# arthurlirui/IRON

Hardware: AMD Instinct MI355X
Metric: Mrays/s sphere-trace+GGX shade, drv/dragon 800x800 (synthetic S0) (higher is better)
Workload: dtype f32

## Files before the change

iron_amd/csrc/getall_rev.hip:

```cpp
#include <stdlib.h>
#include "mlp_h2_rev.h"
#include "h2_setup.h"
#include "shade_args.h"

namespace iron {

template <int T>
__device__ __forceinline__ void pe_contract(const f32x16& g, const float* pe, int half, float& gx, float& gy, float& gz) {
#pragma unroll
    for (int r = 0; r < 16; ++r) {
        const int s = 16 * T + r;
        if (s == 0) {
            if (half) gy += g[r]; else gx += g[r];
        } else if (s == 1) {
            if (!half) gz += g[r];
        } else if (s < 2 + 3 * kSdfPeLevels) {
            const int k = (s - 2) / 3, c = (s - 2) % 3;
            const float f = (float)(1 << k);
            const float v = (half ? f : -f) * pe[s] * g[r];
            if (c == 0) gx += v; else if (c == 1) gy += v; else gz += v;
        }
    }
}

#ifndef IRON_REV_FEAT_NT
#define IRON_REV_FEAT_NT 0
#endif
#ifdef IRON_REV_DEBUG
#define IRON_REV_DUMP(L, BUF)                                                                                              \
    if (dbg == (L) && a.feat_rows && ok) {                                                                                 \
        _Pragma("unroll") for (int t_ = 0; t_ < kHidTiles; ++t_)                                                           \
            _Pragma("unroll") for (int r_ = 0; r_ < 16; ++r_) {                                                            \
                const int s_ = r_ >> 3, j_ = r_ & 7;                                                                       \
                const float v_ = (float)BUF[t_].h[s_][j_] + (float)BUF[t_].l[s_][j_] * kLoInv;                             \
                a.feat_rows[(size_t)li * kHidden + 32 * t_ + (r_ & 3) + 8 * (r_ >> 2) + 4 * half] = v_;                    \
            }                                                                                                              \
    }
#define IRON_REV_DBG_PARAM , int dbg
#else
#define IRON_REV_DUMP(L, BUF)
#define IRON_REV_DBG_PARAM
#endif

__global__ __launch_bounds__(256, 1) void k_sdf_getall_rev_h2(H2StreamDev hs, H2Meta m, GradArgs a, char* __restrict__ park IRON_REV_DBG_PARAM) {
    extern __shared__ __attribute__((aligned(16))) char smem[];
    char* lds = smem;
    const int lane = threadIdx.x & 63;
    const int half = lane >> 5;
    const int wave = __builtin_amdgcn_readfirstlane(threadIdx.x >> 6);
    Ring ring;
    h2_setup(hs, lds, ring);
    ParkBuf pb;
    pb.rsrc = __builtin_amdgcn_make_buffer_rsrc(park + (size_t)blockIdx.x * kParkBytesPerWg, 0, kParkBytesPerWg, 0x00020000);
    pb.voff = lane * 16;
    const int count = a.count_ptr ? *a.count_ptr : a.count;
    const int n_tiles = (count + kTile - 1) / kTile;
    const int n_groups = (n_tiles + 3) / 4;
    const bool want_feat = (a.feat_packed != nullptr) || (a.feat_rows != nullptr);
    const char* bias = lds + kLdsBias;

    for (int g = blockIdx.x; g < n_groups; g += gridDim.x) {
        const int tile = 4 * g + wave;
        const int li = tile * kTile + (lane & 31);
        const bool ok = li < count;
        const int src = ok ? (a.list ? a.list[li] : li) : 0;
        float px = 0.f, py = 0.f, pz = 0.f;
        if (ok) { px = a.x[3 * (size_t)src]; py = a.x[3 * (size_t)src + 1]; pz = a.x[3 * (size_t)src + 2]; }
        const float sx = px * m.scale, sy = py * m.scale, sz = pz * m.scale;

        TileFrag X[kHidTiles], Y[kHidTiles];
        f32x16 hf[kHidTiles];
        HeadFrag hd;
        {
            float pe[kHeadSlots];
#pragma unroll
            for (int i = 0; i < kHeadSlots; ++i) pe[i] = 0.0f;
            head_fill<kSdfPeLevels>(sx, sy, sz, half, pe);
            split_head(pe, hd);
        }
#pragma unroll
        for (int to = 0; to < kHidTiles; ++to) {
            ring.sync();
            const RingStep st = ring.step();
            f32x16 a_hi = zero16(), a_lo = zero16();
            step_head(st.rd, bias, st.wr, st.src, st.hidden, wave, lane, to, true, hd, a_hi, a_lo);
            f32x16 h, P;
            softplus_park_tile(h2_combine(a_hi, a_lo), h, P);
            park_store_tile(pb, park_off(0, to, wave), P);
            split_tile(h, X[to]);
        }
        for (int l = 1; l < 7; l += 2) {
            h2_layer_x<kModeFwd, false, false>(ring, bias + l * 1024, hd, lane, X, Y, hf, pb, l);
            if (l + 1 == 4) h2_layer_x<kModeFwd, true, false>(ring, bias + (l + 1) * 1024, hd, lane, Y, X, hf, pb, l + 1);
            else h2_layer_x<kModeFwd, false, false>(ring, bias + (l + 1) * 1024, hd, lane, Y, X, hf, pb, l + 1);
        }
        h2_layer_x<kModeFwd, false, true>(ring, bias + 7 * 1024, hd, lane, X, Y, hf, pb, 7);
        {
            const float s = (row_dot_lds(lds + kLdsRows, hf, half) + m.b_last) / m.scale;
            if (ok && lane < 32 && a.sdf_out) a.sdf_out[li] = s;
        }
#pragma unroll
        for (int t = 0; t < kHidTiles; ++t) split_tile(hf[t], X[t]);
        {
            const char* fb = bias + 8 * 1024;
            float* dst = (a.feat_packed && tile < n_tiles) ? a.feat_packed + (size_t)tile * (kHidTiles * 16 * 64) : nullptr;
#pragma unroll
            for (int to = 0; to < kHidTiles; ++to) {
                const f32x16 o = h2_plain_tile(ring, fb, lane, to, true, X, pb);
                if (want_feat && !(IRON_REV_ABL & 4)) {
                    if (dst) feat_store_tile<IRON_REV_FEAT_NT != 0>(dst, to, lane, o);
#ifdef IRON_REV_DEBUG
                    if (a.feat_rows && ok && dbg < 0) {
#else
                    if (a.feat_rows && ok) {
#endif
#pragma unroll
                        for (int r = 0; r < 16; ++r) a.feat_rows[(size_t)li * kHidden + 32 * to + (r & 3) + 8 * (r >> 2) + 4 * half] = o[r];
                    }
                }
            }
        }
#pragma unroll
        for (int t = 0; t < kHidTiles; ++t) {
            const f32x16 P = park_load_tile(pb, park_off(7, t, wave));
            f32x16 d = lds_half_tile(lds + kLdsRows, t, half);
#pragma unroll
            for (int i = 0; i < 16; ++i) d[i] *= sigma_from_park(P[i]);
            split_tile(d, Y[t]);
        }
        float gx = 0.f, gy = 0.f, gz = 0.f;
        float pe[kHeadSlots];
#pragma unroll
        for (int i = 0; i < kHeadSlots; ++i) pe[i] = 0.0f;
        if (!(IRON_REV_ABL & 8)) head_fill<kSdfPeLevels>(sx, sy, sz, half, pe);
        IRON_REV_DUMP(7, Y)
        h2_layer_x<kModeBwd, false, false>(ring, bias, hd, lane, Y, X, hf, pb, 6);
        IRON_REV_DUMP(6, X)
        h2_layer_x<kModeBwd, false, false>(ring, bias, hd, lane, X, Y, hf, pb, 5);
        IRON_REV_DUMP(5, Y)
        h2_layer_x<kModeBwd, false, false>(ring, bias, hd, lane, Y, X, hf, pb, 4);
        IRON_REV_DUMP(4, X)
        h2_layer_x<kModeBwd, false, false>(ring, bias, hd, lane, X, Y, hf, pb, 3);
        IRON_REV_DUMP(3, Y)
        {
            const f32x16 g0 = h2_plain_tile(ring, bias, lane, 0, false, X, pb);
            pe_contract<0>(g0, pe, half, gx, gy, gz);
            const f32x16 g1 = h2_plain_tile(ring, bias, lane, 1, false, X, pb);
            pe_contract<1>(g1, pe, half, gx, gy, gz);
        }
        h2_layer_x<kModeBwd, false, false>(ring, bias, hd, lane, Y, X, hf, pb, 2);
        IRON_REV_DUMP(2, X)
        h2_layer_x<kModeBwd, false, false>(ring, bias, hd, lane, X, Y, hf, pb, 1);
        IRON_REV_DUMP(1, Y)
        h2_layer_x<kModeBwd, false, false>(ring, bias, hd, lane, Y, X, hf, pb, 0);
        IRON_REV_DUMP(0, X)
        {
            const f32x16 g0 = h2_plain_tile(ring, bias, lane, 0, false, X, pb);
            pe_contract<0>(g0, pe, half, gx, gy, gz);
            const f32x16 g1 = h2_plain_tile(ring, bias, lane, 1, false, X, pb);
            pe_contract<1>(g1, pe, half, gx, gy, gz);
        }
        gx += __shfl_xor(gx, 32, 64);
        gy += __shfl_xor(gy, 32, 64);
        gz += __shfl_xor(gz, 32, 64);
        if (ok && lane < 32 && a.grad_out) {
            a.grad_out[3 * (size_t)li] = gx; a.grad_out[3 * (size_t)li + 1] = gy; a.grad_out[3 * (size_t)li + 2] = gz;
        }
    }
    ring.drain();
}

size_t getall_rev_park_bytes(int64_t n_points) {
    const int64_t groups = (n_points + 127) / 128;
    const int64_t cus = cu_total();
    return (size_t)(groups < cus ? (groups > 0 ? groups : 1) : cus) * kParkBytesPerWg;
}

bool getall_rev_usable(const iron_net* sdf) {
    static int on = -1;
    if (on < 0) {
        const char* e = getenv("IRON_GETALL");
        on = (e && e[0] == 'f') ? 0 : 1;
    }
    return on == 1 && h2_sdf_usable(sdf) && sdf->h2_rev_blob != nullptr;
}

int launch_sdf_getall_rev(const iron_net* sdf, const GradArgs& a, int64_t max_tiles, void* park, size_t park_bytes, hipStream_t st) {
    static bool attr = false;
    if (!attr) {
        IRON_HIP_TRY(hipFuncSetAttribute((const void*)k_sdf_getall_rev_h2, hipFuncAttributeMaxDynamicSharedMemorySize, kLdsH2Total));
        attr = true;
    }
    H2Meta m;
    m.n_hidden_layers = sdf->sdf.n_hidden_layers; m.skip_layer = sdf->sdf.skip_layer; m.scale = sdf->sdf.scale; m.b_last = sdf->sdf.b_last;
    const int64_t groups = (max_tiles + 3) / 4;
    const int64_t cus = cu_budget();
    int64_t grid = groups < cus ? (groups > 0 ? groups : 1) : cus;
    const int64_t cap = (int64_t)(park_bytes / kParkBytesPerWg);
    if (!park || cap < 1) return IRON_ERR_WORKSPACE;
    if (grid > cap) grid = cap;
    if (((uintptr_t)park & 15) != 0) return IRON_ERR_BAD_ARG;
    ProfScope ps(IRON_PROF_SDF_GRAD, st);
#ifdef IRON_REV_DEBUG
    const char* de = getenv("IRON_REV_DEBUG_LAYER");
    hipLaunchKernelGGL(k_sdf_getall_rev_h2, dim3((unsigned)grid), dim3(256), kLdsH2Total, st, sdf->h2_rev, m, a, (char*)park, de ? atoi(de) : -1);
#else
    hipLaunchKernelGGL(k_sdf_getall_rev_h2, dim3((unsigned)grid), dim3(256), kLdsH2Total, st, sdf->h2_rev, m, a, (char*)park);
#endif
    IRON_HIP_TRY(hipGetLastError());
    return IRON_OK;
}

}
```

iron_amd/csrc/mlp_core.h:

```cpp
#pragma once
#include "iron_common.h"

namespace iron {

typedef float f32x16 __attribute__((ext_vector_type(16)));
typedef float f32x4 __attribute__((ext_vector_type(4)));
typedef int i32x4 __attribute__((ext_vector_type(4)));

template <bool NT = false>
__device__ __forceinline__ void feat_store_tile(float* __restrict__ tile_base, int t, int lane, const f32x16& o) {
    f32x4* p = reinterpret_cast<f32x4*>(tile_base) + (size_t)(t * 4) * 64 + lane;
#pragma unroll
    for (int q = 0; q < 4; ++q) {
        f32x4 v;
        v[0] = o[4 * q]; v[1] = o[4 * q + 1]; v[2] = o[4 * q + 2]; v[3] = o[4 * q + 3];
        if (NT) __builtin_nontemporal_store(v, p + q * 64);
        else p[q * 64] = v;
    }
}
__device__ __forceinline__ f32x16 feat_load_tile(const float* __restrict__ tile_base, int t, int lane) {
    const float4* p = reinterpret_cast<const float4*>(tile_base) + (size_t)(t * 4) * 64 + lane;
    f32x16 v;
#pragma unroll
    for (int q = 0; q < 4; ++q) {
        const float4 x = p[q * 64];
        v[4 * q] = x.x; v[4 * q + 1] = x.y; v[4 * q + 2] = x.z; v[4 * q + 3] = x.w;
    }
    return v;
}

#ifndef IRON_WQ_DEPTH
#define IRON_WQ_DEPTH 4
#endif

__device__ __forceinline__ f32x16 mfma32(float a, float b, f32x16 c) {
    return __builtin_amdgcn_mfma_f32_32x32x2f32(a, b, c, 0, 0, 0);
}

struct WStream {
    __amdgpu_buffer_rsrc_t rsrc;
    int v_lane;
    int v_half;
    __device__ __forceinline__ void init(const void* blob, uint32_t bytes, int lane) {
        rsrc = __builtin_amdgcn_make_buffer_rsrc(const_cast<void*>(blob), 0, (int)bytes, 0x00020000);
        v_lane = lane * 16;
        v_half = (lane >> 5) * 64;
    }
    __device__ __forceinline__ f32x4 frag(uint32_t s_off) const {
        return __builtin_bit_cast(f32x4, __builtin_amdgcn_raw_buffer_load_b128(rsrc, v_lane, (int)s_off, 0));
    }
    __device__ __forceinline__ f32x4 half_row(uint32_t s_off) const {
        return __builtin_bit_cast(f32x4, __builtin_amdgcn_raw_buffer_load_b128(rsrc, v_half, (int)s_off, 0));
    }
};

template <bool FAST>
__device__ __forceinline__ float softplus100(float z) {
    if constexpr (FAST) {
        const float e = __builtin_amdgcn_exp2f(__builtin_fabsf(z) * -144.26950408889634f);
        return __builtin_fmaf(__builtin_amdgcn_logf(1.0f + e), 0.0069314718055994531f, fmaxf(z, 0.0f));
    } else {
        const float t = z * 100.0f;
        const float s = log1pf(expf(t)) / 100.0f;
        return t > 20.0f ? z : s;
    }
}

__device__ __forceinline__ float softplus100_grad(float z) {
    const float t = z * 100.0f;
    const float s = 1.0f / (1.0f + expf(-t));
    return t > 20.0f ? 1.0f : s;
}

__device__ __forceinline__ f32x16 load_half_tile(const WStream& ws, uint32_t base, int tile) {
    const uint32_t o = base + (uint32_t)tile * 128u;
    const f32x4 b0 = ws.half_row(o), b1 = ws.half_row(o + 16), b2 = ws.half_row(o + 32), b3 = ws.half_row(o + 48);
    f32x16 v;
    v[0] = b0.x; v[1] = b0.y; v[2] = b0.z; v[3] = b0.w;
    v[4] = b1.x; v[5] = b1.y; v[6] = b1.z; v[7] = b1.w;
    v[8] = b2.x; v[9] = b2.y; v[10] = b2.z; v[11] = b2.w;
    v[12] = b3.x; v[13] = b3.y; v[14] = b3.z; v[15] = b3.w;
    return v;
}

template <int LEVELS>
__device__ __forceinline__ void head_fill(float vx, float vy, float vz, int half, float* slots) {
    slots[0] = half ? vy : vx;
    slots[1] = half ? 0.0f : vz;
#pragma unroll
    for (int k = 0; k < LEVELS; ++k) {
        const float f = (float)(1 << k);
        float s, c;
        sincosf(vx * f, &s, &c); slots[2 + 3 * k + 0] = half ? c : s;
        sincosf(vy * f, &s, &c); slots[2 + 3 * k + 1] = half ? c : s;
        sincosf(vz * f, &s, &c); slots[2 + 3 * k + 2] = half ? c : s;
    }
}

template <int LEVELS>
__device__ __forceinline__ void head_fill4(float vx, float vy, float vz, float vw, int half, float* slots) {
    slots[0] = half ? vy : vx;
    slots[1] = half ? vw : vz;
    const float v[4] = {vx, vy, vz, vw};
#pragma unroll
    for (int k = 0; k < LEVELS; ++k) {
        const float f = (float)(1 << k);
#pragma unroll
        for (int c = 0; c < 4; ++c) {
            float s, cs;
            sincosf(v[c] * f, &s, &cs);
            slots[2 + 4 * k + c] = half ? cs : s;
        }
    }
}

__device__ __forceinline__ void mfma_quad(const f32x4& a0, const f32x4& a1, float b0, float b1, float b2, float b3,
                                          f32x16& acc0, f32x16& acc1) {
    acc0 = mfma32(a0.x, b0, acc0);
    acc1 = mfma32(a1.x, b0, acc1);
    acc0 = mfma32(a0.y, b1, acc0);
    acc1 = mfma32(a1.y, b1, acc1);
    acc0 = mfma32(a0.z, b2, acc0);
    acc1 = mfma32(a1.z, b2, acc1);
    acc0 = mfma32(a0.w, b3, acc0);
    acc1 = mfma32(a1.w, b3, acc1);
}

template <int NQ>
__device__ __forceinline__ void dense_head_pair(const WStream& ws, uint32_t base, int pair, const float* head,
                                                f32x16& acc0, f32x16& acc1) {
    const uint32_t o = base + (uint32_t)pair * (NQ * 2048u);
    constexpr int kChunk = NQ <= 6 ? NQ : 6;
#pragma unroll
    for (int q0 = 0; q0 < NQ; q0 += kChunk) {
        f32x4 a0[kChunk], a1[kChunk];
#pragma unroll
        for (int q = 0; q < kChunk; ++q) {
            if (q0 + q < NQ) {
                a0[q] = ws.frag(o + (q0 + q) * 2048u);
                a1[q] = ws.frag(o + (q0 + q) * 2048u + 1024u);
            }
        }
#pragma unroll
        for (int q = 0; q < kChunk; ++q) {
            if (q0 + q < NQ)
                mfma_quad(a0[q], a1[q], head[4 * (q0 + q)], head[4 * (q0 + q) + 1], head[4 * (q0 + q) + 2], head[4 * (q0 + q) + 3],
                          acc0, acc1);
        }
    }
}

struct WQueue {
    static constexpr int D = IRON_WQ_DEPTH;
    f32x4 a0[D], a1[D];
    __device__ __forceinline__ void prime(const WStream& ws, uint32_t base) {
#pragma unroll
        for (int d = 0; d < D; ++d) {
            a0[d] = ws.frag(base + d * 2048u);
            a1[d] = ws.frag(base + d * 2048u + 1024u);
        }
    }
};

#ifndef IRON_SCHED_MASK
#define IRON_SCHED_MASK 0x6
#endif

template <int PAIR>
__device__ __forceinline__ void dense_hidden_pair(const WStream& ws, uint32_t base, WQueue& wq,
                                                  const f32x16 (&in)[kHidTiles], f32x16& acc0, f32x16& acc1) {
#pragma unroll
    for (int s = 0; s < 32; ++s) {
        constexpr int D = WQueue::D;
        const int g = PAIR * 32 + s;
        const int slot = g % D;
        const f32x4 x0 = wq.a0[slot], x1 = wq.a1[slot];
        wq.a0[slot] = ws.frag(base + (uint32_t)(g + D) * 2048u);
        wq.a1[slot] = ws.frag(base + (uint32_t)(g + D) * 2048u + 1024u);
// ... 128 lines not shown
```

iron_amd/csrc/mlp_h2.h:

```cpp
#pragma once
#include "iron_common.h"
#include "mlp_core.h"
#include "lds_dma.h"

#ifndef IRON_H2_STAMP
#define IRON_H2_STAMP 0
#endif
#ifndef IRON_H2_ASM_DMA
#define IRON_H2_ASM_DMA 0
#endif
#ifndef IRON_H2_FRAG_AHEAD
#define IRON_H2_FRAG_AHEAD 1
#endif
#ifndef IRON_H2_RING_AHEAD
#define IRON_H2_RING_AHEAD 3
#endif
#ifndef IRON_H2_SPREAD
#define IRON_H2_SPREAD 1
#endif
#ifndef IRON_H2_ABL
#define IRON_H2_ABL 0
#endif
#ifndef IRON_H2_ROT_ISSUE
#define IRON_H2_ROT_ISSUE 0
#endif

namespace iron {

typedef _Float16 half8 __attribute__((ext_vector_type(8)));
typedef _Float16 half2v __attribute__((ext_vector_type(2)));

constexpr int kRingSlots = 4;
constexpr int kSlotBytes = 32768;
constexpr int kRingBytes = kRingSlots * kSlotBytes;
constexpr int kRingAhead = IRON_H2_RING_AHEAD;
constexpr int kLoadsPerSlot = 8;
constexpr float kLoScale = 2048.0f;
constexpr float kLoInv = 1.0f / 2048.0f;
constexpr int kHeadSlots = 24;
constexpr int kHeadKSteps = 3;

constexpr int kLdsRing = 0;
constexpr int kLdsBias = kRingBytes;
constexpr int kLdsBiasBytes = 9 * 1024;
constexpr int kLdsRows = kLdsBias + kLdsBiasBytes;
constexpr int kLdsRowsBytes = 3 * 1024;
constexpr int kLdsTable = kLdsRows + kLdsRowsBytes;
constexpr int kLdsTableBytes = 1024;
constexpr int kLdsMisc = kLdsTable + kLdsTableBytes;
constexpr int kLdsMiscBytes = 256;
constexpr int kLdsH2Total = kLdsMisc + kLdsMiscBytes;

constexpr int kLdsStamp = kLdsH2Total;
constexpr int kStampSteps = 72;
constexpr int kStampFirst = 144;
constexpr int kLdsStampBytes = 4 * kStampSteps * 8 * 8;
__device__ __forceinline__ void h2_stamp(unsigned long long* rec, int k) {
#if IRON_H2_STAMP
    if (rec) {
        const unsigned long long t = __builtin_readcyclecounter();
        if ((threadIdx.x & 63) == 0) rec[k] = t;
    }
    __builtin_amdgcn_sched_barrier(0);
#endif
}

__device__ __forceinline__ f32x16 mfma_h(half8 a, half8 b, f32x16 c) {
    return __builtin_amdgcn_mfma_f32_32x32x16_f16(a, b, c, 0, 0, 0);
}

typedef _Float16 f16x2 __attribute__((ext_vector_type(2)));
typedef unsigned int u32x4 __attribute__((ext_vector_type(4)));

__device__ __forceinline__ void split2(float x0, float x1, unsigned& hi, unsigned& lo) {
    f16x2 h;
    h[0] = (_Float16)x0;
    h[1] = (_Float16)x1;
    f16x2 l;
    l[0] = (_Float16)((x0 - (float)h[0]) * kLoScale);
    l[1] = (_Float16)((x1 - (float)h[1]) * kLoScale);
    hi = __builtin_bit_cast(unsigned, h);
    lo = __builtin_bit_cast(unsigned, l);
}

struct TileFrag {
    half8 h[2];
    half8 l[2];
};

__device__ __forceinline__ void split8(const float* v, half8& h, half8& l) {
    u32x4 hh, ll;
#pragma unroll
    for (int i = 0; i < 4; ++i) {
        unsigned a, b;
        split2(v[2 * i], v[2 * i + 1], a, b);
        hh[i] = a;
        ll[i] = b;
    }
    h = __builtin_bit_cast(half8, hh);
    l = __builtin_bit_cast(half8, ll);
}

__device__ __forceinline__ void split_tile(const f32x16& v, TileFrag& t) {
#pragma unroll
// ... 468 lines not shown
                                                const HeadFrag* hd2 = nullptr, const float* __restrict__ init = nullptr) {
    static_assert(!INIT || HEAD > 0, "the partial sums are added on top of the head product");
    static_assert(!(LAST && DEFER), "the last layer ends in f32 tiles");
    const int wave = ring.wave;
    f32x16 acc[2][2];
    TileFrag dummy_out;
    f32x16 dummy_hf;
#define IRON_H2_TILE(TO)                                                                                                   \
    if constexpr ((TO) < NT) {                                                                                             \
        constexpr int P = (TO) & 1, Q = P ^ 1;                                                                             \
        acc[P][0] = zero16();                                                                                              \
        acc[P][1] = zero16();                                                                                              \
        f32x16 part;                                                                                                       \
        if constexpr (INIT) {                                                                                              \
            _Pragma("unroll") for (int r = 0; r < 16; ++r) part[r] = init[((TO) * 16 + r) * 64 + lane];                    \
        }                                                                                                                  \
        if constexpr (HEAD >= 1) {                                                                                         \
            ring.sync();                                                                                                   \
            const RingStep sh = ring.step();                                                                               \
            step_head(sh.rd, bias, sh.wr, sh.src, sh.hidden, wave, lane, TO, true, hd, acc[P][0], acc[P][1]);              \
        }                                                                                                                  \
        if constexpr (HEAD >= 2) {                                                                                         \
            ring.sync();                                                                                                   \
            const RingStep sh = ring.step();                                                                               \
            step_head(sh.rd, bias, sh.wr, sh.src, sh.hidden, wave, lane, TO, false, *hd2, acc[P][0], acc[P][1]);           \
        }                                                                                                                  \
        if constexpr (INIT) {                                                                                              \
            _Pragma("unroll") for (int r = 0; r < 16; ++r) acc[P][0][r] += part[r];                                        \
        }                                                                                                                  \
        ring.sync();                                                                                                       \
        const RingStep st = ring.step();                                                                                   \
        if constexpr ((TO) == 0 && CARRY)                                                                                  \
            step_hidden<FAST, 1, ACT, true>(st.rd, bias, st.wr, st.src, st.hidden, wave, lane, TO, !HEAD, in, acc[P][0],   \
                                            acc[P][1], c_hi, c_lo, dummy_out, dummy_hf, st.rec);                           \
        else if constexpr ((TO) == 0)                                                                                      \
            step_hidden<FAST, 0, ACT>(st.rd, bias, st.wr, st.src, st.hidden, wave, lane, TO, !HEAD, in, acc[P][0], acc[P][1],   \
                                 acc[Q][0], acc[Q][1], dummy_out, dummy_hf, st.rec);                                       \
        else if constexpr (LAST)                                                                                           \
            step_hidden<FAST, 2, ACT>(st.rd, bias, st.wr, st.src, st.hidden, wave, lane, TO, !HEAD, in, acc[P][0], acc[P][1],   \
                                 acc[Q][0], acc[Q][1], dummy_out, hf[(TO) > 0 ? (TO) - 1 : 0], st.rec);                    \
        else                                                                                                               \
            step_hidden<FAST, 1, ACT>(st.rd, bias, st.wr, st.src, st.hidden, wave, lane, TO, !HEAD, in, acc[P][0], acc[P][1],   \
                                 acc[Q][0], acc[Q][1], out[(TO) > 0 ? (TO) - 1 : 0], dummy_hf, st.rec);                    \
    }
    IRON_H2_TILE(0) IRON_H2_TILE(1) IRON_H2_TILE(2) IRON_H2_TILE(3)
    IRON_H2_TILE(4) IRON_H2_TILE(5) IRON_H2_TILE(6) IRON_H2_TILE(7)
#undef IRON_H2_TILE
    static_assert(NT % 2 == 0 && NT >= 2 && NT <= kHidTiles, "the last tile sits in accumulator set 1");
    if constexpr (DEFER) {
        c_hi = acc[1][0];
        c_lo = acc[1][1];
    } else if constexpr (ACT == 0) {
        if constexpr (LAST) hf[NT - 1] = softplus_tile<FAST>(h2_combine(acc[1][0], acc[1][1]));
        else h2_epilogue_split<FAST>(acc[1][0], acc[1][1], out[NT - 1]);
    } else if constexpr (ACT == 1) {
        if constexpr (LAST) hf[NT - 1] = relu_tile_nan(h2_combine(acc[1][0], acc[1][1]));
        else split_tile(relu_tile_nan(h2_combine(acc[1][0], acc[1][1])), out[NT - 1]);
    } else {
        if constexpr (LAST) hf[NT - 1] = h2_combine(acc[1][0], acc[1][1]);
        else split_tile(h2_combine(acc[1][0], acc[1][1]), out[NT - 1]);
    }
}

__device__ __forceinline__ float row_dot_lds(const char* __restrict__ row, const f32x16 (&h)[kHidTiles], int half) {
    float s = 0.0f;
#pragma unroll
    for (int t = 0; t < kHidTiles; ++t) {
        const f32x16 w = lds_half_tile(row, t, half);
#pragma unroll
        for (int r = 0; r < 16; ++r) s = fmaf(w[r], h[t][r], s);
    }
    return s + __shfl_xor(s, 32, 64);
}

template <bool FAST, bool DEFER_TILES = true>
__device__ __forceinline__ void sdf_hidden_stack_h2(Ring& ring, const char* lds, int n_hidden_layers, int skip_layer,
                                                    float scale, float x, float y, float z, int lane,
                                                    f32x16 (&hf)[kHidTiles]) {
    const int half = lane >> 5;
    const int wave = ring.wave;
    float pe[kHeadSlots];
#pragma unroll
    for (int i = 0; i < kHeadSlots; ++i) pe[i] = 0.0f;
    head_fill<kSdfPeLevels>(x * scale, y * scale, z * scale, half, pe);
    HeadFrag hd;
    split_head(pe, hd);

    TileFrag X[kHidTiles], Y[kHidTiles];
#pragma unroll
    for (int to = 0; to < kHidTiles; ++to) {
        ring.sync();
        const RingStep st = ring.step();
        f32x16 a_hi = zero16(), a_lo = zero16();
        step_head(st.rd, lds + kLdsBias, st.wr, st.src, st.hidden, wave, lane, to, true, hd, a_hi, a_lo);
        h2_epilogue_split<FAST>(a_hi, a_lo, X[to]);
    }
    f32x16 c_hi, c_lo;
    constexpr bool D = DEFER_TILES;
    for (int l = 1; l + 1 < n_hidden_layers - 1; l += 2) {
        const char* bias_a = lds + kLdsBias + l * 1024;
        const char* bias_b = bias_a + 1024;
        if (l == 1) h2_hidden_layer<FAST, false, false, 0, false, D>(ring, bias_a, hd, lane, X, Y, hf, c_hi, c_lo);
        else h2_hidden_layer<FAST, false, false, 0, D, D>(ring, bias_a, hd, lane, X, Y, hf, c_hi, c_lo);
        if (l + 1 == skip_layer) h2_hidden_layer<FAST, true, false, 0, D, D>(ring, bias_b, hd, lane, Y, X, hf, c_hi, c_lo);
        else h2_hidden_layer<FAST, false, false, 0, D, D>(ring, bias_b, hd, lane, Y, X, hf, c_hi, c_lo);
    }
    h2_hidden_layer<FAST, false, true, 0, D, false>(ring, lds + kLdsBias + (n_hidden_layers - 1) * 1024, hd, lane, X, Y, hf, c_hi, c_lo);
}

#ifndef IRON_H1_NO_EPI
#define IRON_H1_NO_EPI 0
#endif
constexpr int kH1PointTiles = 2;

struct Epi1State {
    float z[16], e[16];
    u32x4 oh[2];
};

constexpr int kEpi1Ops = 104;
constexpr int kEpi1OpsF32 = 96;

template <bool F32>
__device__ __forceinline__ void epi1_op(Epi1State& st, int op, const f32x16& p) {
    constexpr float kC1 = 144.26950408889634f;
    constexpr float kC2 = 0.0069314718055994531f;
    constexpr int kHalf = F32 ? 48 : 52;
    const int h = op / kHalf, lo = op % kHalf;
#if IRON_H1_NO_EPI
    if (lo >= 48) {
        const int q = 4 * h + lo - 48;
        st.oh[q >> 2][q & 3] = __builtin_bit_cast(unsigned, cvt_pk_rn(p[2 * q], p[2 * q + 1]));
    }
    if (lo >= 40 && lo < 48) st.z[8 * h + lo - 40] = p[8 * h + lo - 40];
    return;
#endif
    if (lo >= 48) {
        const int q = 4 * h + lo - 48;
        unsigned u = __builtin_bit_cast(unsigned, cvt_pk_rn(st.z[2 * q], st.z[2 * q + 1]));
        pin1u(u);
        st.oh[q >> 2][q & 3] = u;
        return;
    }
    const int stage = lo >> 3, i = 8 * h + (lo & 7);
    if (stage == 0) { st.e[i] = __builtin_fabsf(p[i]) * -kC1; pin1(st.e[i]); }
    else if (stage == 1) { st.e[i] = __builtin_amdgcn_exp2f(st.e[i]); pin1(st.e[i]); }
    else if (stage == 2) { st.e[i] = 1.0f + st.e[i]; pin1(st.e[i]); }
    else if (stage == 3) { st.e[i] = __builtin_amdgcn_logf(st.e[i]); pin1(st.e[i]); }
    else if (stage == 4) { st.z[i] = relu_med3(p[i]); pin1(st.z[i]); }
    else { st.z[i] = __builtin_fmaf(st.e[i], kC2, st.z[i]); pin1(st.z[i]); }
}

struct TileH {
    half8 h[2];
};

struct HeadH {
    half8 h[kHeadKSteps];
};

__device__ __forceinline__ void tile_from_epi(const Epi1State& es, TileH& t) {
#pragma unroll
    for (int s = 0; s < 2; ++s) t.h[s] = __builtin_bit_cast(half8, es.oh[s]);
}

__device__ __forceinline__ void row_dot_tile(const char* __restrict__ row, int t, int half, const float* z, float& s) {
    const f32x16 w = lds_half_tile(row, t, half);
#pragma unroll
    for (int r = 0; r < 16; ++r) s = fmaf(w[r], z[r], s);
}

#ifndef IRON_H1_FRAG_AHEAD
#define IRON_H1_FRAG_AHEAD 1
#endif
constexpr int kH1Ahead = IRON_H1_FRAG_AHEAD;
static_assert(kH1Ahead == 1 || kH1Ahead == 2, "IRON_H1_FRAG_AHEAD: 1 or 2");
struct H1Pre {
    half8 f[kH1Ahead];
};

__device__ __forceinline__ const char* h1_slot(Ring& ring, H1Pre& pre, int lane) {
    ring.sync();
    ring.b_take = __builtin_amdgcn_readfirstlane(ring.b_take);
    const RingStep st = ring.step();
#pragma unroll
// ... 230 lines not shown
```

iron_amd/csrc/shade.hip:

```cpp
#include "mlp_h2.h"
#include "h2_setup.h"
#include "ggx_core.h"
#include "shade_args.h"

namespace iron {

#ifndef IRON_FAST_SOFTPLUS
#define IRON_FAST_SOFTPLUS 1
#endif
constexpr bool kFastActS = IRON_FAST_SOFTPLUS != 0;

template <bool FAST>
__device__ __forceinline__ void softplus100_both(float z, float& h, float& s) {
    if constexpr (FAST) {
        const float u = __builtin_amdgcn_exp2f(__builtin_fabsf(z) * -144.26950408889634f);
        const float w = 1.0f + u;
        h = __builtin_fmaf(__builtin_amdgcn_logf(w), 0.0069314718055994531f, fmaxf(z, 0.0f));
        s = (z >= 0.0f ? 1.0f : u) * __builtin_amdgcn_rcpf(w);
    } else {
        const float t = z * 100.0f;
        const float e = expf(t);
        const float l = log1pf(e) / 100.0f;
        const float sg = e / (e + 1.0f);
        const bool lin = t > 20.0f;
// ... 66 lines not shown
    {                                                                                               \
        f32x16 a0 = is_value ? load_half_tile(ws, bb, 2 * P) : zero_tile();                         \
        f32x16 a1 = is_value ? load_half_tile(ws, bb, 2 * P + 1) : zero_tile();                     \
        if (with_head) dense_head_pair<kSdfHeadQuads>(ws, hb, P, head, a0, a1);                     \
        if (l > 0) dense_hidden_pair<P>(ws, wb, wq, h, a0, a1);                                     \
        if (is_value) {                                                                             \
            _Pragma("unroll") for (int r = 0; r < 16; ++r) {                                        \
                float hv, sv;                                                                       \
                softplus100_both<kFastActS>(a0[r], hv, sv);                                         \
                a0[r] = hv;                                                                         \
                sbuf[((2 * P) * 16 + r) * 64 + lane] = sv;                                          \
                softplus100_both<kFastActS>(a1[r], hv, sv);                                         \
                a1[r] = hv;                                                                         \
                sbuf[((2 * P + 1) * 16 + r) * 64 + lane] = sv;                                      \
            }                                                                                       \
        }                                                                                           \
        o[2 * P] = a0;                                                                              \
        o[2 * P + 1] = a1;                                                                          \
    }
            IRON_GPAIR(0) IRON_GPAIR(1) IRON_GPAIR(2) IRON_GPAIR(3)
#undef IRON_GPAIR
            __syncthreads();
            if (!is_value) {
#pragma unroll
                for (int t = 0; t < kHidTiles; ++t)
#pragma unroll
                    for (int r = 0; r < 16; ++r) o[t][r] *= sbuf[(t * 16 + r) * 64 + lane];
            }
#pragma unroll
            for (int t = 0; t < kHidTiles; ++t) h[t] = o[t];
        }

        if (is_value) {
            const float s = (row_dot(ws, net.w_last, h) + net.b_last) / net.scale;
            if (ok && lane < 32 && a.sdf_out) a.sdf_out[li] = s;
            if ((a.feat_packed || a.feat_rows) && net.w_feat) {
                f32x16 o[kHidTiles];
                WQueue wf;
                wf.prime(ws, net.w_feat);
                hidden_layer<IdentityAct, 1>(ws, net.w_feat, net.b_feat, false, 0u, nullptr, wf, h, o, IdentityAct());
                if (a.feat_packed) {
                    float* dst = a.feat_packed + (size_t)tile * kSBufFloats;
#pragma unroll
                    for (int t = 0; t < kHidTiles; ++t) feat_store_tile(dst, t, lane, o[t]);
                }
                if (a.feat_rows && ok) {
#pragma unroll
                    for (int t = 0; t < kHidTiles; ++t)
#pragma unroll
                        for (int r = 0; r < 16; ++r)
                            a.feat_rows[(size_t)li * kHidden + 32 * t + (r & 3) + 8 * (r >> 2) + 4 * half] = o[t][r];
                }
            }
        } else {
            const float g = row_dot(ws, net.w_last, h);
            if (ok && lane < 32 && a.grad_out) a.grad_out[3 * (size_t)li + axis] = g;
        }
        __syncthreads();
    }
}

constexpr int kLdsSbuf = kLdsH2Total;
constexpr int kLdsGradTotal = kLdsH2Total + 8192;

#if defined(IRON_GRAD_VARIANT) && (IRON_GRAD_VARIANT & 1)
#define IRON_GRAD_ACT(Z, H, S) { H = (Z); S = 1.0f; }
#else
#define IRON_GRAD_ACT(Z, H, S) softplus100_both<kFastActS>(Z, H, S)
#endif

__device__ __forceinline__ void lds_publish_barrier() {
    asm volatile("s_waitcnt lgkmcnt(0)" ::: "memory");
    __builtin_amdgcn_s_barrier();
}

__device__ __forceinline__ float sdf_value_or_tangent_h2(Ring& ring, char* lds, float* sbuf, const H2Meta& m, float px, float py,
                                                         float pz, bool is_value, int axis, int wave, int lane,
                                                         TileFrag (&in)[kHidTiles], TileFrag (&out)[kHidTiles]) {
    const int half = lane >> 5;
    const float sx = px * m.scale, sy = py * m.scale, sz = pz * m.scale;
    float head[kHeadSlots];
#pragma unroll
    for (int i = 0; i < kHeadSlots; ++i) head[i] = 0.0f;
    if (is_value) head_fill<kSdfPeLevels>(sx, sy, sz, half, head);
    else head_fill_tangent<kSdfPeLevels>(sx, sy, sz, axis, half, head);
    HeadFrag hd;
    split_head(head, hd);
    TileFrag dummy_out;
    f32x16 dummy_hf;
    f32x16 p_hi = zero16(), p_lo = zero16();
    for (int l = 0; l < m.n_hidden_layers; ++l) {
        const bool last = (l == m.n_hidden_layers - 1);
        const bool with_head = (l == 0) || (l == m.skip_layer);
        const char* bias = lds + kLdsBias + l * 1024;
        if (l > 0) {
#pragma unroll
            for (int t = 0; t < kHidTiles; ++t) in[t] = out[t];
        }
#define IRON_GTILE(TO)                                                                                                  \
    {                                                                                                                   \
        f32x16 a_hi = zero16(), a_lo = zero16();                                                                        \
        if (with_head) {                                                                                                \
            ring.sync();                                                                                                \
            const RingStep sh = ring.step();                                                                            \
            step_head(sh.rd, bias, sh.wr, sh.src, sh.hidden, wave, lane, TO, false, hd, a_hi, a_lo);                    \
        }                                                                                                               \
        if (l > 0) {                                                                                                    \
            ring.sync();                                                                                                \
            const RingStep st = ring.step();                                                                            \
            step_hidden<kFastActS, 0>(st.rd, bias, st.wr, st.src, st.hidden, wave, lane, TO, false, in, a_hi, a_lo,     \
                                      a_hi, a_lo, dummy_out, dummy_hf);                                                 \
        }                                                                                                               \
        if (is_value) {                                                                                                 \
             \
             \
            f32x16 zt = h2_combine(a_hi, a_lo);                                                                         \
            const f32x16 bt = lds_half_tile(bias, TO, half);                                                            \
            float* sb = sbuf + ((TO) & 1) * (16 * 64);                                                                  \
            _Pragma("unroll") for (int r = 0; r < 16; ++r) {                                                            \
                float hv, sv;                                                                                           \
                IRON_GRAD_ACT(zt[r] + bt[r], hv, sv);                                                                   \
                zt[r] = hv;                                                                                             \
                sb[r * 64 + lane] = sv;                                                                                 \
            }                                                                                                           \
            asm volatile("s_waitcnt lgkmcnt(0)" ::: "memory");                                                          \
            if (last) out[TO] = __builtin_bit_cast(TileFrag, zt);                                                       \
            else split_tile(zt, out[TO]);                                                                               \
        } else {                                                                                                        \
             \
            if ((TO) > 0) IRON_GTANGENT_FINISH((TO) - 1)                                                                \
            p_hi = a_hi;                                                                                                \
            p_lo = a_lo;                                                                                                \
        }                                                                                                               \
    }
#define IRON_GTANGENT_FINISH(T)                                                                                         \
    {                                                                                                                   \
        f32x16 zt = h2_combine(p_hi, p_lo);                                                                             \
        const float* sb = sbuf + ((T) & 1) * (16 * 64);                                                                 \
        _Pragma("unroll") for (int r = 0; r < 16; ++r) zt[r] *= sb[r * 64 + lane];                                      \
        if (last) out[T] = __builtin_bit_cast(TileFrag, zt);                                                            \
        else split_tile(zt, out[T]);                                                                                    \
    }
        IRON_GTILE(0) IRON_GTILE(1) IRON_GTILE(2) IRON_GTILE(3) IRON_GTILE(4) IRON_GTILE(5) IRON_GTILE(6) IRON_GTILE(7)
        lds_publish_barrier();
        if (!is_value) IRON_GTANGENT_FINISH(7)
#undef IRON_GTANGENT_FINISH
#undef IRON_GTILE
    }
    f32x16 hf[kHidTiles];
#pragma unroll
    for (int t = 0; t < kHidTiles; ++t) hf[t] = __builtin_bit_cast(f32x16, out[t]);
    const float d = row_dot_lds(lds + kLdsRows, hf, half);
    return is_value ? (d + m.b_last) / m.scale : d;
}

__global__ __launch_bounds__(256, 1) void k_sdf_grad_h2(H2StreamDev hs, H2Meta m, GradArgs a) {
    extern __shared__ __attribute__((aligned(16))) char smem[];
    char* lds = smem;
    const int lane = threadIdx.x & 63;
    const int half = lane >> 5;
    const int wave = __builtin_amdgcn_readfirstlane(threadIdx.x >> 6);
    const bool is_value = wave == 0;
    const int axis = wave - 1;
    Ring ring;
    h2_setup(hs, lds, ring);
    float* sbuf = reinterpret_cast<float*>(lds + kLdsSbuf);
    const int count = a.count_ptr ? *a.count_ptr : a.count;
// ... 170 lines not shown
        if (ok) {
            px = a.points[3 * (size_t)pi]; py = a.points[3 * (size_t)pi + 1]; pz = a.points[3 * (size_t)pi + 2];
            if (a.normals) { nx = a.normals[3 * (size_t)ai]; ny = a.normals[3 * (size_t)ai + 1]; nz = a.normals[3 * (size_t)ai + 2]; }
            if (a.normalise) {
                const float nn = sqrtf((nx * nx + ny * ny) + nz * nz) + 1e-10f;
                nx = nx / nn; ny = ny / nn; nz = nz / nn;
            }
            if (a.neg_normal_view) { vx = -nx; vy = -ny; vz = -nz; }
            else if (a.view) { vx = a.view[3 * (size_t)ai]; vy = a.view[3 * (size_t)ai + 1]; vz = a.view[3 * (size_t)ai + 2]; }
        }
        float head[4 * NQ];
#pragma unroll
        for (int i = 0; i < 4 * NQ; ++i) head[i] = 0.0f;
        int base = 0;
        head_fill<LP>(px, py, pz, half, head + base);
        base += head_slots(LP);
        if constexpr (HAS_VIEW) { head_fill<LV>(vx, vy, vz, half, head + base); base += head_slots(LV); }
        if constexpr (HAS_NRM) { head_fill<0>(nx, ny, nz, half, head + base); base += 2; }

        f32x16 h[kHidTiles];
        load_feature_tiles(a, tile, ai, ok, lane, half, h);

        WQueue wq;
        wq.prime(ws, net.w_feat0);
        for (int l = 0, blk = 0; l < net.n_hidden_layers; ++l) {
            const uint32_t bb = net.bias + (uint32_t)l * (kF4PerBiasLayer * 16u);
            f32x16 o[kHidTiles];
            if (l == 0) {
                hidden_layer<ReluAct, NQ>(ws, net.w_feat0, bb, true, net.w_head0, head, wq, h, o, ReluAct());
            } else if (HAS_SKIP && l == net.skip_layer) {
                hidden_layer<IdentityAct, NQ>(ws, net.w_hid + (uint32_t)(blk++) * (kF4PerHidLayer * 16u), bb, true, net.w_head_skip, head,
                                              wq, h, o, IdentityAct());
                load_feature_tiles(a, tile, ai, ok, lane, half, h);
                hidden_layer_accumulate<ReluAct>(ws, net.w_hid + (uint32_t)(blk++) * (kF4PerHidLayer * 16u), wq, h, o, ReluAct());
            } else {
                hidden_layer<ReluAct, NQ>(ws, net.w_hid + (uint32_t)(blk++) * (kF4PerHidLayer * 16u), bb, false, net.w_head0, head, wq, h, o,
                                          ReluAct());
            }
#pragma unroll
            for (int t = 0; t < kHidTiles; ++t) h[t] = o[t];
        }
        for (int c = 0; c < net.d_out; ++c) {
            float v = row_dot(ws, net.w_last + (uint32_t)c * (kF4PerBiasLayer * 16u), h) + net.b_last[c];
            v = net.output_scale * (v + net.output_bias);
            if (net.squeeze_out) v = net.squeeze_out_scale * (1.0f / (1.0f + expf(-v)));
            if (ok && lane < 32) a.out[(size_t)li * net.d_out + c] = v;
        }
    }
}

template <int LP, int LV, bool HAS_VIEW, bool HAS_NRM>
__global__ __launch_bounds__(256, 1) void k_material_h2(H2StreamDev hs, RenderNetDev net, MatArgs a) {
    extern __shared__ __attribute__((aligned(16))) char smem[];
    char* lds = smem;
    const int lane = threadIdx.x & 63;
    const int half = lane >> 5;
    const int wave = __builtin_amdgcn_readfirstlane(threadIdx.x >> 6);
    Ring ring;
    h2_setup(hs, lds, ring);
    const int count = a.count_ptr ? *a.count_ptr : a.count;
    const int n_tiles = (count + kTile - 1) / kTile;
    const int n_groups = (n_tiles + 3) / 4;
    for (int g = blockIdx.x; g < n_groups; g += gridDim.x) {
        const int tile = g * 4 + wave;
        const int li = tile * kTile + (lane & 31);
        const bool ok = li < count;
        const int pi = ok ? (a.list ? a.list[li] : li) : 0;
        const int ai = ok ? (a.list_order_aux ? li : pi) : 0;
        float px = 0.f, py = 0.f, pz = 0.f, nx = 0.f, ny = 0.f, nz = 1.f, vx = 0.f, vy = 0.f, vz = 0.f;
        if (ok) {
            px = a.points[3 * (size_t)pi]; py = a.points[3 * (size_t)pi + 1]; pz = a.points[3 * (size_t)pi + 2];
            if (a.normals) { nx = a.normals[3 * (size_t)ai]; ny = a.normals[3 * (size_t)ai + 1]; nz = a.normals[3 * (size_t)ai + 2]; }
            if (a.normalise) {
                const float nn = sqrtf((nx * nx + ny * ny) + nz * nz) + 1e-10f;
                nx = nx / nn; ny = ny / nn; nz = nz / nn;
            }
            if (a.neg_normal_view) { vx = -nx; vy = -ny; vz = -nz; }
            else if (a.view) { vx = a.view[3 * (size_t)ai]; vy = a.view[3 * (size_t)ai + 1]; vz = a.view[3 * (size_t)ai + 2]; }
        }
        float head[kHeadSlots];
#pragma unroll
        for (int i = 0; i < kHeadSlots; ++i) head[i] = 0.0f;
        int base = 0;
        head_fill<LP>(px, py, pz, half, head + base);
        base += head_slots(LP);
        if constexpr (HAS_VIEW) { head_fill<LV>(vx, vy, vz, half, head + base); base += head_slots(LV); }
        if constexpr (HAS_NRM) { head_fill<0>(nx, ny, nz, half, head + base); base += 2; }
        HeadFrag hd;
        split_head(head, hd);

        TileFrag in[kHidTiles], out[kHidTiles];
        f32x16 hf[kHidTiles];
        {
            const bool tile_ok = tile < n_tiles;
            const float* src = (a.feat_packed && tile_ok) ? a.feat_packed + (size_t)tile * kSBufFloats : nullptr;
#pragma unroll
            for (int t = 0; t < kHidTiles; ++t) {
                f32x16 v = zero16();
                if (src) {
                    v = feat_load_tile(src, t, lane);
                } else if (a.feat_rows && ok) {
                    const float4* row = reinterpret_cast<const float4*>(a.feat_rows + (size_t)ai * kHidden);
#pragma unroll
                    for (int q = 0; q < 4; ++q) {
                        const float4 w4 = row[(32 * t + 8 * q + 4 * half) >> 2];
                        v[4 * q] = w4.x; v[4 * q + 1] = w4.y; v[4 * q + 2] = w4.z; v[4 * q + 3] = w4.w;
                    }
                }
                split_tile(v, out[t]);
            }
        }
        f32x16 c_hi, c_lo;
        h2_hidden_layer<true, true, false, 1, false, true>(ring, lds + kLdsBias, hd, lane, out, in, hf, c_hi, c_lo);
        for (int l = 1; l + 1 < net.n_hidden_layers - 1; l += 2) {
            h2_hidden_layer<true, false, false, 1, true, true>(ring, lds + kLdsBias + l * 1024, hd, lane, in, out, hf, c_hi, c_lo);
            h2_hidden_layer<true, false, false, 1, true, true>(ring, lds + kLdsBias + (l + 1) * 1024, hd, lane, out, in, hf, c_hi, c_lo);
        }
        h2_hidden_layer<true, false, true, 1, true, false>(ring, lds + kLdsBias + (net.n_hidden_layers - 1) * 1024, hd, lane, in, out, hf,
                                                           c_hi, c_lo);
        for (int c = 0; c < net.d_out; ++c) {
            float v = row_dot_lds(lds + kLdsRows + c * 1024, hf, half) + net.b_last[c];
            v = net.output_scale * (v + net.output_bias);
            if (net.squeeze_out) v = net.squeeze_out_scale * (1.0f / (1.0f + expf(-v)));
            if (ok && lane < 32) a.out[(size_t)li * net.d_out + c] = v;
        }
    }
    ring.drain();
}

template <int LP, int LV, bool HAS_VIEW, bool HAS_NRM>
__global__ __launch_bounds__(256, 1) void k_material_h2_skip(H2StreamDev hs, RenderNetDev net, MatArgs a, float* __restrict__ scratch) {
    static_assert(HeadCfg<LP, LV, HAS_VIEW, HAS_NRM>::kSlots > kHeadSlots && HeadCfg<LP, LV, HAS_VIEW, HAS_NRM>::kSlots <= 2 * kHeadSlots, "two head slots");
    extern __shared__ __attribute__((aligned(16))) char smem[];
    char* lds = smem;
    const int lane = threadIdx.x & 63;
    const int half = lane >> 5;
    const int wave = __builtin_amdgcn_readfirstlane(threadIdx.x >> 6);
    Ring ring;
    h2_setup(hs, lds, ring);
    float* part = scratch + ((size_t)blockIdx.x * 4 + wave) * (kHidTiles * 16 * 64);
    const int count = a.count_ptr ? *a.count_ptr : a.count;
    const int n_tiles = (count + kTile - 1) / kTile;
    const int n_groups = (n_tiles + 3) / 4;
    for (int g = blockIdx.x; g < n_groups; g += gridDim.x) {
        const int tile = g * 4 + wave;
        const int li = tile * kTile + (lane & 31);
        const bool ok = li < count;
        const int pi = ok ? (a.list ? a.list[li] : li) : 0;
        const int ai = ok ? (a.list_order_aux ? li : pi) : 0;
        float px = 0.f, py = 0.f, pz = 0.f, nx = 0.f, ny = 0.f, nz = 1.f, vx = 0.f, vy = 0.f, vz = 0.f;
        if (ok) {
            px = a.points[3 * (size_t)pi]; py = a.points[3 * (size_t)pi + 1]; pz = a.points[3 * (size_t)pi + 2];
            if (a.normals) { nx = a.normals[3 * (size_t)ai]; ny = a.normals[3 * (size_t)ai + 1]; nz = a.normals[3 * (size_t)ai + 2]; }
            if (a.normalise) {
                const float nn = sqrtf((nx * nx + ny * ny) + nz * nz) + 1e-10f;
                nx = nx / nn; ny = ny / nn; nz = nz / nn;
            }
            if (a.neg_normal_view) { vx = -nx; vy = -ny; vz = -nz; }
            else if (a.view) { vx = a.view[3 * (size_t)ai]; vy = a.view[3 * (size_t)ai + 1]; vz = a.view[3 * (size_t)ai + 2]; }
        }
        HeadFrag hd, hd2;
        {
            float head[2 * kHeadSlots];
#pragma unroll
            for (int i = 0; i < 2 * kHeadSlots; ++i) head[i] = 0.0f;
            int base = 0;
            head_fill<LP>(px, py, pz, half, head + base);
            base += head_slots(LP);
            if constexpr (HAS_VIEW) { head_fill<LV>(vx, vy, vz, half, head + base); base += head_slots(LV); }
// ... 548 lines not shown
```

Before: 19.11.

## Share positional-encoding sincos across wave halves and defer last layer-0 tile epilogue

Adds head_fill_paired. Each wave half now computes sincos for only half the frequency levels: the low half takes the low levels, the high half takes the upshifted levels. A v_permlane32_swap then exchanges sin and cos between the halves, so each lane gets the values it needs while evaluating half as many transcendentals. Separately, in the sphere-trace MLP path, the last layer-0 tile's accumulators are kept as deferred c_hi/c_lo and finished inside the first hidden layer, which should overlap the epilogue with later work. The inline asm uses an explicit s_nop hazard guard and is specific to gfx950. It assumes the frequency level count is even and that the slot layout matches the original per-half sin/cos assignment.

```diff
diff --git a/iron_amd/csrc/getall_rev.hip b/iron_amd/csrc/getall_rev.hip
--- a/iron_amd/csrc/getall_rev.hip
+++ b/iron_amd/csrc/getall_rev.hip
@@ -75,7 +75,7 @@
             float pe[kHeadSlots];
 #pragma unroll
             for (int i = 0; i < kHeadSlots; ++i) pe[i] = 0.0f;
-            head_fill<kSdfPeLevels>(sx, sy, sz, half, pe);
+            head_fill_paired<kSdfPeLevels>(sx, sy, sz, half, pe);
             split_head(pe, hd);
         }
 #pragma unroll
@@ -132,7 +132,7 @@
         float pe[kHeadSlots];
 #pragma unroll
         for (int i = 0; i < kHeadSlots; ++i) pe[i] = 0.0f;
-        if (!(IRON_REV_ABL & 8)) head_fill<kSdfPeLevels>(sx, sy, sz, half, pe);
+        if (!(IRON_REV_ABL & 8)) head_fill_paired<kSdfPeLevels>(sx, sy, sz, half, pe);
         IRON_REV_DUMP(7, Y)
         h2_layer_x<kModeBwd, false, false>(ring, bias, hd, lane, Y, X, hf, pb, 6);
         IRON_REV_DUMP(6, X)
diff --git a/iron_amd/csrc/mlp_core.h b/iron_amd/csrc/mlp_core.h
--- a/iron_amd/csrc/mlp_core.h
+++ b/iron_amd/csrc/mlp_core.h
@@ -94,6 +94,34 @@
         sincosf(vx * f, &s, &c); slots[2 + 3 * k + 0] = half ? c : s;
         sincosf(vy * f, &s, &c); slots[2 + 3 * k + 1] = half ? c : s;
         sincosf(vz * f, &s, &c); slots[2 + 3 * k + 2] = half ? c : s;
+    }
+}
+
+#ifndef IRON_H2_PE_SHARE
+#define IRON_H2_PE_SHARE 1
+#endif
+template <int LEVELS>
+__device__ __forceinline__ void head_fill_paired(float vx, float vy, float vz, int half, float* slots) {
+    if constexpr (IRON_H2_PE_SHARE != 0 && LEVELS >= 2 && LEVELS % 2 == 0) {
+        constexpr int LH = LEVELS / 2;
+        slots[0] = half ? vy : vx;
+        slots[1] = half ? 0.0f : vz;
+        const float up = half ? (float)(1 << LH) : 1.0f;
+        const float v[3] = {vx, vy, vz};
+#pragma unroll
+        for (int k = 0; k < LH; ++k) {
+            const float f = (float)(1 << k) * up;
+#pragma unroll
+            for (int c = 0; c < 3; ++c) {
+                float s, co;
+                sincosf(v[c] * f, &s, &co);
+                asm volatile("s_nop 1\n\tv_permlane32_swap_b32 %0, %1" : "+v"(s), "+v"(co));
+                slots[2 + 3 * k + c] = s;
+                slots[2 + 3 * (k + LH) + c] = co;
+            }
+        }
+    } else {
+        head_fill<LEVELS>(vx, vy, vz, half, slots);
     }
 }
 
diff --git a/iron_amd/csrc/mlp_h2.h b/iron_amd/csrc/mlp_h2.h
--- a/iron_amd/csrc/mlp_h2.h
+++ b/iron_amd/csrc/mlp_h2.h
@@ -20,6 +20,9 @@
 #endif
 #ifndef IRON_H2_ABL
 #define IRON_H2_ABL 0
+#endif
+#ifndef IRON_H2_DEFER_L0
+#define IRON_H2_DEFER_L0 1
 #endif
 #ifndef IRON_H2_ROT_ISSUE
 #define IRON_H2_ROT_ISSUE 0
@@ -654,25 +657,31 @@
     float pe[kHeadSlots];
 #pragma unroll
     for (int i = 0; i < kHeadSlots; ++i) pe[i] = 0.0f;
-    head_fill<kSdfPeLevels>(x * scale, y * scale, z * scale, half, pe);
+    head_fill_paired<kSdfPeLevels>(x * scale, y * scale, z * scale, half, pe);
     HeadFrag hd;
     split_head(pe, hd);
 
     TileFrag X[kHidTiles], Y[kHidTiles];
+    f32x16 c_hi, c_lo;
+    constexpr bool D = DEFER_TILES;
+    constexpr bool D0 = DEFER_TILES && IRON_H2_DEFER_L0 != 0;
 #pragma unroll
     for (int to = 0; to < kHidTiles; ++to) {
         ring.sync();
         const RingStep st = ring.step();
         f32x16 a_hi = zero16(), a_lo = zero16();
         step_head(st.rd, lds + kLdsBias, st.wr, st.src, st.hidden, wave, lane, to, true, hd, a_hi, a_lo);
-        h2_epilogue_split<FAST>(a_hi, a_lo, X[to]);
-    }
-    f32x16 c_hi, c_lo;
-    constexpr bool D = DEFER_TILES;
+        if (D0 && to == kHidTiles - 1) {
+            c_hi = a_hi;
+            c_lo = a_lo;
+        } else {
+            h2_epilogue_split<FAST>(a_hi, a_lo, X[to]);
+        }
+    }
     for (int l = 1; l + 1 < n_hidden_layers - 1; l += 2) {
         const char* bias_a = lds + kLdsBias + l * 1024;
         const char* bias_b = bias_a + 1024;
-        if (l == 1) h2_hidden_layer<FAST, false, false, 0, false, D>(ring, bias_a, hd, lane, X, Y, hf, c_hi, c_lo);
+        if (l == 1) h2_hidden_layer<FAST, false, false, 0, D0, D>(ring, bias_a, hd, lane, X, Y, hf, c_hi, c_lo);
         else h2_hidden_layer<FAST, false, false, 0, D, D>(ring, bias_a, hd, lane, X, Y, hf, c_hi, c_lo);
         if (l + 1 == skip_layer) h2_hidden_layer<FAST, true, false, 0, D, D>(ring, bias_b, hd, lane, Y, X, hf, c_hi, c_lo);
         else h2_hidden_layer<FAST, false, false, 0, D, D>(ring, bias_b, hd, lane, Y, X, hf, c_hi, c_lo);
diff --git a/iron_amd/csrc/shade.hip b/iron_amd/csrc/shade.hip
--- a/iron_amd/csrc/shade.hip
+++ b/iron_amd/csrc/shade.hip
@@ -172,7 +172,7 @@
     float head[kHeadSlots];
 #pragma unroll
     for (int i = 0; i < kHeadSlots; ++i) head[i] = 0.0f;
-    if (is_value) head_fill<kSdfPeLevels>(sx, sy, sz, half, head);
+    if (is_value) head_fill_paired<kSdfPeLevels>(sx, sy, sz, half, head);
     else head_fill_tangent<kSdfPeLevels>(sx, sy, sz, axis, half, head);
     HeadFrag hd;
     split_head(head, hd);
@@ -509,9 +509,9 @@
 #pragma unroll
         for (int i = 0; i < kHeadSlots; ++i) head[i] = 0.0f;
         int base = 0;
-        head_fill<LP>(px, py, pz, half, head + base);
+        head_fill_paired<LP>(px, py, pz, half, head + base);
         base += head_slots(LP);
-        if constexpr (HAS_VIEW) { head_fill<LV>(vx, vy, vz, half, head + base); base += head_slots(LV); }
+        if constexpr (HAS_VIEW) { head_fill_paired<LV>(vx, vy, vz, half, head + base); base += head_slots(LV); }
         if constexpr (HAS_NRM) { head_fill<0>(nx, ny, nz, half, head + base); base += 2; }
         HeadFrag hd;
         split_head(head, hd);
```

Result: no change. 19.28 (median of 6 runs) (+0.9%).
